# microsoft/ConfigNet

Hardware: AMD Instinct MI355X
Metric: train-step images/sec at 256x256 (G+D fwd+bwd) (higher is better)
Workload: dtype f32; 1 GPU; ConfigNet second-stage iteration (D + synth-D + latent-D + G + EMA), 256x256, batch 16 per GPU, fp32, Keras-Adam; global_batch=16, resolution=256, latent_dim=145, parallelism=dp1, losses_finite=True

## Files before the change

### confignet_amd/_lib.py

```python
import ctypes
import os

_HERE = os.path.dirname(os.path.abspath(__file__))
LIB_PATH = os.environ.get("CN_LIB") or os.path.join(_HERE, "libconfignet_hip.so")


class CnSumJob(ctypes.Structure):
    _fields_ = [("src", ctypes.c_void_p), ("dst", ctypes.c_void_p), ("count", ctypes.c_longlong), ("parts", ctypes.c_int),
                ("accumulate", ctypes.c_int)]


class CnDepthJob(ctypes.Structure):
    _fields_ = [("a", ctypes.c_void_p), ("b", ctypes.c_void_p), ("c", ctypes.c_void_p), ("m", ctypes.c_int), ("n", ctypes.c_int),
                ("k", ctypes.c_int), ("lda", ctypes.c_int), ("ldb", ctypes.c_int), ("ldc", ctypes.c_int)]


class CnRowsJob(ctypes.Structure):
    _fields_ = [("a", ctypes.c_void_p), ("b", ctypes.c_void_p), ("c", ctypes.c_void_p), ("bias", ctypes.c_void_p), ("mask", ctypes.c_void_p)] + \
               [(n_, ctypes.c_int) for n_ in ("m", "n", "k", "lda", "ldb", "ldc", "tb", "act", "accumulate")] + [("slope", ctypes.c_float)]


class CnGanJob(ctypes.Structure):
    _fields_ = [("s", ctypes.c_void_p), ("out", ctypes.c_void_p), ("gout", ctypes.c_void_p), ("n", ctypes.c_int), ("label", ctypes.c_float)]


class CnConvGeom(ctypes.Structure):
    _fields_ = [(n, ctypes.c_int) for n in (
        "nd", "n", "in_d", "in_h", "in_w", "cin", "out_d", "out_h", "out_w", "cout",
        "k_d", "k_h", "k_w", "s_d", "s_h", "s_w", "dl_d", "dl_h", "dl_w", "p_d", "p_h", "p_w", "up")]


CN_F32, CN_BF16 = 0, 1
CN_U8 = 2
CN_EUNSUPPORTED = -3


class ConfigNetHipError(RuntimeError):
    pass


if not os.path.exists(LIB_PATH):
    raise ImportError(
        "confignet_amd: %s is missing -- build it with `python confignet_amd/build.py` "
        "(or __graft_entry__.build()).  There is no CPU/PyTorch fallback." % LIB_PATH)

lib = ctypes.CDLL(LIB_PATH)

_p = ctypes.c_void_p
_i = ctypes.c_int
_f = ctypes.c_float
_z = ctypes.c_size_t
_G = ctypes.POINTER(CnConvGeom)

SIGNATURES = {
    "cn_version": [],
    "cn_conv_fwd": [_G, _p, _p, _p, _p, _i, _f, _p],
    "cn_conv_fwd_res": [_G, _p, _p, _p, _p, _p, _i, _f, _p],
    "cn_conv_fwd_stats": [_G, _p, _p, _p, _p, _i, _f, _p, _i, _f, _p],
    "cn_scale_columns_segments": [_p, _p, _p, _p, _i, _z, _p],
    "cn_conv_weight_tflip": [_p, _p, _i, _i, _i, _p],
    "cn_conv_dgrad": [_G, _p, _p, _p, _p],
    "cn_conv_dgrad_w": [_G, _p, _p, _p, _p],
    "cn_conv_dgrad_w_res": [_G, _p, _p, _p, _p, _p],
    "cn_conv_dgrad_w_mask": [_G, _p, _p, _p, _p, _p, _p, _p, _p],
    "cn_bn_fold_bwd_chunks": [],
    "cn_bn_fold_bwd": [_p, _i, _i, _p, _p, _p, _p, _p, _p, _p, _p, _i, _p],
    "cn_conv_wgrad_thin_partials": [],
    "cn_conv_wgrad_thin": [_G, _p, _p, _p, _p, _i, _p],
    "cn_conv_wgrad": [_G, _p, _p, _p, _i, _p],
    "cn_conv_wgrad_workspace_bytes": [_G],
    "cn_conv_wgrad_ws": [_G, _p, _p, _p, _i, _p, _z, _p],
    "cn_conv_wgrad_ws_slabs": [_G, _p, _p, _p, _i, _p, _z, ctypes.POINTER(_i), _p],
    "cn_conv_wgrad_dt_workspace_bytes": [_G, _i, _i, ctypes.POINTER(_z)],
    "cn_conv_wgrad_dt": [_G, _p, _i, _p, _i, _p, _i, _p, _z, ctypes.POINTER(_i), _p],
    "cn_conv_wgrad_plan": [_G, _i, _i, _i, ctypes.c_uint, _i, ctypes.POINTER(ctypes.c_longlong)],
    "cn_conv_wgrad_grouped": [_i, _p, _p, _p, _p, _p, _p, _p, _i, _p, _p],
    "cn_conv_wgrad_grouped_plan": [_i, _p, _i, _p, _p],
    "cn_sum_parts_grouped": [_p, _i, _p],
    "cn_gemm_depth_grouped": [_p, _i, _p],
    "cn_gan_loss_grouped": [_p, _i, _i, _p],
    "cn_gemm_rows_grouped": [_p, _i, _p],
    "cn_gemm_rows_grouped_k": [_p, _i, _p],
    "cn_gemm_rows_grouped_plan": [_p, _i, ctypes.POINTER(_i), _i, ctypes.POINTER(_i)],
    "cn_conv_tune": [_i, _i, ctypes.c_long],
    "cn_conv_fwd_plan": [_G, _i, _i, _i, _i, _i, _i, _i, ctypes.POINTER(ctypes.c_int * 8)],
    "cn_conv_fwd_plan_ep": [_G, _i, _i, _i, _i, _i, _i, _i, _i, ctypes.POINTER(ctypes.c_int * 8)],
    "cn_conv_loop_select": [_i, _i, _i, _i],
    "cn_fwd2_col_block": [_i, _i, _i, _i, _i, _i],
    "cn_conv_fwd_dt": [_p, _p, _i, _p, _p, _p, _i, _i, _f, _p],
    "cn_conv_dgrad_dt": [_p, _p, _i, _p, _p, _i, _p],
    "cn_conv_wgrad_c3_partials": [],
    "cn_conv_wgrad_c3": [_p, _p, _p, _i, _p, _p, _i, _p],
    "cn_conv_wino_filter": [_p, _p, _i, _i, _i, _p],
    "cn_conv_fwd_wino": [_i, _i, _i, _i, _i, _p, _p, _p, _p, _i, _f, _p],
    "cn_conv_fwd_wino_ep": [_i, _i, _i, _i, _i, _p, _p, _p, _p, _p, _p, _p],
    "cn_conv_fwd_wino4": [_i, _i, _i, _i, _i, _p, _p, _p, _p, _i, _f, _p],
    "cn_conv_fwd_wino4_ep": [_i, _i, _i, _i, _i, _p, _p, _p, _p, _i, _f, _i, _p, _p, _p, _p, _i, _f, _p],
    "cn_conv_wino4_filter": [_p, _p, _i, _i, _i, _p],
    "cn_sumpool2": [_p, _p, _i, _i, _i, _i, _i, _i, _i, _p],
    "cn_gemm": [_i, _i, _i, _i, _i, _p, _i, _p, _i, _p, _i, _p, _i, _f, _p],
    "cn_gemm_plan": [_i] * 10 + [ctypes.POINTER(ctypes.c_int * 9)],
    "cn_nc_reduce4": [_p, _p, _i, _i, _i, _f, _i, _i, _p],
    "cn_nc_reduce": [_p, _p, _p, _p, _i, _i, _i, _i, _f, _i, _p],
    "cn_nc_reduce_plan": [_i, _i, _i, _i, _i, _i, ctypes.POINTER(ctypes.c_int * 8)],
    "cn_nc_lin2": [_p, _p, _p, _p, _p, _p, _p, _p, _i, _i, _i, _i, _i, _f, _i, _p],
    "cn_nc_rows_plan": [ctypes.c_longlong, _i, _i, ctypes.POINTER(ctypes.c_int * 2)],
    "cn_norm_coef_fwd": [_i, _p, _p, _p, _p, _p, _p, _p, _p, _i, _i, _i, _f, _p, _i, _p],
    "cn_norm_coef_bwd": [_i, _p, _p, _p, _p, _p, _p, _p, _p, _p, _p, _i, _i, _i, _f, _p],
    "cn_dual_tail_coef_fwd": [_p] * 13 + [_i, _i, _i, _f, _i, _i, _p],
    "cn_dual_tail_coef_bwd": [_p] * 13 + [ctypes.POINTER(ctypes.c_void_p), _i, _i, _i, _f, _i, _i, _p],
    "cn_dual_tail_gx": [_p] * 12 + [_i, _i, _i, _f, _i, _i, _p],
    "cn_dual_tail_gx_tx": [_p] * 18 + [_i, _i, _i, _f, _i, _i, _i, _p],
    "cn_norm_apply": [_i, _i] + [_p] * 13 + [_i, _i, _i, _f, _i, _f, _i, _p],
    "cn_nc_reduce_hxt": [_p, _p, _p, _p, _i, _i, _i, _f, _i, _i, _i, _p],
    "cn_zero": [_p, ctypes.c_size_t, _p],
    "cn_set_deterministic": [_i],
    "cn_get_deterministic": [],
    "cn_det_release_stream": [_p],
    "cn_gemm_acc": [_i, _i, _i, _i, _i, _p, _i, _p, _i, _p, _i, _p],
    "cn_sum_rows_into": [_p, _p, _i, _i, _i, _p],
    "cn_bn_act_bwd": [_p, _p, _p, _p, _p, _p, _p, _p, _i, _i, _i, _i, _i, _i, _p],
    "cn_nc_reduce_dact": [_p, _p, _p, _p, _p, _i, _i, _i, _i, _f, _i, _i, _p],
    "cn_act_fwd": [_p, _p, _z, _i, _f, _i, _p],
    "cn_act_bwd": [_p, _p, _p, _z, _i, _f, _i, _p],
    "cn_act_bwd_bias": [_p, _p, _p, _p, _i, _i, _i, _i, _f, _i, _i, _p],
    "cn_axpby": [_p, _p, _p, _z, _f, _f, _i, _p],
    "cn_mul": [_p, _p, _p, _z, _i, _p],
    "cn_sqdiff_sum": [_p, _p, _p, _z, _f, _i, _p],
    "cn_row_sumsq": [_p, _p, _i, _z, _p],
    "cn_row_scale": [_p, _p, _p, _i, _z, _f, _i, _p],
    "cn_row_scale_diff": [_p, _p, _p, _p, _i, ctypes.c_size_t, _f, _i, _p],
    "cn_tap_bwd": [_p, _p, _p, _p, _p, _i, ctypes.c_size_t, _f, _i, _f, _i, _p],
    "cn_maxpool2_bwd_act": [_p, _p, _p, _p, _f, _p, _i, _i, _i, _i, _i, _i, _p],
    "cn_stream_plan": [_i, _i, ctypes.c_longlong, _z, _i, _i, _i, _i, _i, _i, ctypes.c_uint, _i, ctypes.POINTER(ctypes.c_longlong * 4)],
    "cn_stream_plan_ptrs": [_i, _i, _i, ctypes.c_longlong, _z, _i, _i, _i, _i, _i, _i, ctypes.POINTER(ctypes.c_void_p * 4), _i, ctypes.POINTER(ctypes.c_longlong * 4)],
    "cn_stream_last_plan": [ctypes.POINTER(ctypes.c_longlong * 5)],
    "cn_masked_diff": [_p, _p, _p, _p, _z, _i, _p],
    "cn_maxpool_fwd": [_p, _p, _i, _i, _i, _i, _i, _i, _i, _i, _p],
    "cn_maxpool_bwd": [_p, _p, _p, _i, _i, _i, _i, _i, _i, _i, _i, _p],
    "cn_avgpool3_same": [_p, _p, _i, _i, _i, _i, _i, _p],
    "cn_dwconv3x3_fwd": [_p, _p, _p, _p, _i, _i, _i, _i, _i, _i, _f, _p],
    "cn_image_preprocess": [_p, _i, _p, _i, _i, _i, _i, _i, _i, _f, _f, _p],
    "cn_dwconv3x3_dgrad": [_p, _p, _p, _i, _i, _i, _i, _i, _p],
    "cn_dwconv3x3_wgrad_slices": [_i, _i, _i, _i, _i],
    "cn_dwconv3x3_wgrad": [_p, _p, _p, _i, _i, _i, _i, _i, _i, _p],
    "cn_bn_train_coef": [_p] * 12 + [ctypes.c_longlong, _i, _f, ctypes.c_double, _i, _p],
    "cn_bn_train_apply": [_p, _p, _p, _p, ctypes.c_longlong, _i, _i, _p],
# ... 50 lines not shown
```

### confignet_amd/build.py

```python
import os
import subprocess
import sys

CSRC = os.path.join(os.path.dirname(os.path.abspath(__file__)), "csrc")
LIB = os.path.join(os.path.dirname(os.path.abspath(__file__)), "libconfignet_hip.so")
SOURCES = ["prof.hip", "igemm_conv.hip", "small_conv.hip", "conv_dispatch.hip", "igemm_bf16.hip", "upfold.hip", "winograd.hip", "winograd4.hip", "c3_wgrad.hip", "thin_wgrad.hip", "wgrad2.hip", "fwd2.hip", "gemm.hip", "elementwise.hip", "norm_coef.hip", "rotate3d.hip", "depthwise.hip", "bn_train.hip", "hdri.hip", "dataset.hip"]
FLAGS = ["--offload-arch=gfx950", "-O3", "-std=c++17", "-fPIC", "-munsafe-fp-atomics", "-Wall"]


def _stale(target, deps):
    if not os.path.exists(target):
        return True
    t = os.path.getmtime(target)
    return any(os.path.getmtime(d) > t for d in deps)


def build_library(force=False, verbose=True):
    hipcc = os.environ.get("HIPCC", "/opt/rocm/bin/hipcc")
    headers = [os.path.join(CSRC, f) for f in os.listdir(CSRC) if f.endswith(".h")]
    headers.append(os.path.join(os.path.dirname(CSRC), "..", "include", "confignet_hip.h"))
    objs = []
    procs = []
    for src in SOURCES:
        s = os.path.join(CSRC, src)
        o = os.path.join(CSRC, src.replace(".hip", ".o"))
        objs.append(o)
        if force or _stale(o, [s] + headers):
            cmd = [hipcc] + FLAGS + ["-c", s, "-o", o]
            if verbose:
                print(" ".join(cmd), flush=True)
            procs.append((src, subprocess.Popen(cmd)))
    for src, p in procs:
        if p.wait() != 0:
            raise RuntimeError("hipcc failed on %s" % src)
    if force or procs or _stale(LIB, objs):
        cmd = [hipcc, "--offload-arch=gfx950", "-shared", "-fPIC", "-o", LIB] + objs
        if verbose:
            print(" ".join(cmd), flush=True)
        subprocess.check_call(cmd)
    return LIB


if __name__ == "__main__":
    build_library(force="--force" in sys.argv)
    print(LIB)
```

### confignet_amd/functional.py

```python
import contextlib

import torch
from torch.autograd import Function

from . import ops
from .ops import ACT_LRELU, ACT_NONE, ACT_RELU, ACT_TANH, ConvSpec

_INPUT_GRADS_ONLY = False
FUSED_TAIL_STATS = True
FUSED_R1_TAIL = True
BN_BWD_FUSED = True


@contextlib.contextmanager
def input_grads_only():
    global _INPUT_GRADS_ONLY
    prev, _INPUT_GRADS_ONLY = _INPUT_GRADS_ONLY, True
    try:
        yield
    finally:
        _INPUT_GRADS_ONLY = prev


class _RefuseFn(Function):
# ... 19 lines not shown
    outs = list(outs)
    for i, w in zip(live, wrapped):
        outs[i] = w
    return tuple(outs)


def _cg(t):
    return t if t.is_contiguous() else t.contiguous()


def _bias_grad(gy, first_order, sink=None):
    if first_order:
        return ops.bias_grad(gy.detach(), sink=sink)
    return NcSumDotFn.apply(gy, None, True)[0].reshape(-1)


class ConvFn(Function):

    @staticmethod
    def forward(ctx, x, w, bias, spec, act, slope):
        x, w = _cg(x), _cg(w)
        g = spec.geom(tuple(x.shape), w.shape[-1])
        if ops.upfold_ok(g):
            wf, _, gd, _ = ops.upfold_prepare(w, g)
            y = ops.conv_fwd(x, wf, bias, gd, act, slope)
            ops.prof_note_saved(ops.upfold_saved_flops(g))
        else:
            y = ops.conv_fwd(x, w, bias, g, act, slope)
        ctx.save_for_backward(x, w, y if act != ACT_NONE else None)
        ctx.g, ctx.act, ctx.slope, ctx.has_bias = g, act, slope, bias is not None
        ctx.bias_ref = bias if (bias is not None and bias.requires_grad) else None
        return y

    @staticmethod
    def backward(ctx, gy):
        x, w, y = ctx.saved_tensors
        gy = _cg(gy)
        gb_fused = None
        first_order = not torch.is_grad_enabled()
        want_w = ctx.needs_input_grad[1] and not _INPUT_GRADS_ONLY
        want_b = ctx.has_bias and ctx.needs_input_grad[2] and not _INPUT_GRADS_ONLY
        w_slot = ops.sink_for(w) if (first_order and want_w) else None
        b_slot = ops.sink_for(ctx.bias_ref) if (first_order and want_b and ctx.bias_ref is not None) else None
        if ctx.act != ACT_NONE:
            if not first_order:
                raise RuntimeError("double backward through a fused-activation conv is not supported; "
                                   "use conv(..., act=ACT_NONE) + lrelu()")
            if want_b:
                gy, gb_fused = ops.act_bwd_bias(gy, y, ctx.act, ctx.slope, sink=b_slot)
            else:
                gy = ops.act_bwd(gy, y, ctx.act, ctx.slope)
        elif want_b and b_slot is not None:
            ops.bias_grad(gy.detach(), sink=b_slot)
        gx = gw = gb = None
        if want_b and b_slot is None:
            gb = gb_fused if gb_fused is not None else _bias_grad(gy, first_order)
        if ops.upfold_ok(ctx.g) and first_order:
            _, wd, _, g2 = ops.upfold_prepare(w, ctx.g)
            if ctx.needs_input_grad[0]:
                gx = ops.conv_fwd(gy, wd, None, g2)
                ops.prof_note_saved(ops.upfold_saved_flops(ctx.g))
            if want_w:
                if w_slot is not None:
                    ops.sink_upfold_wgrad(gy, x, g2, tuple(wd.shape), ctx.g, tuple(w.shape), w_slot)
                else:
                    gw = ops.upfold_wgrad(ops.conv_wgrad(gy, x, g2, tuple(wd.shape)), ctx.g, tuple(w.shape))
                ops.prof_note_saved(ops.upfold_saved_flops(ctx.g))
            return gx, gw, gb, None, None, None
        if ctx.needs_input_grad[0]:
            gx = ConvDgradFn.apply(gy, w, ctx.g)
        if want_w:
            if w_slot is not None:
                ops.sink_conv_wgrad(x, gy, ctx.g, tuple(w.shape), w_slot)
            else:
                gw = ConvWgradFn.apply(x, gy, ctx.g, tuple(w.shape))
        return gx, gw, gb, None, None, None


class ConvDgradFn(Function):

    @staticmethod
    def forward(ctx, gy, w, g):
        gy = _cg(gy)
        gu = ops.conv_dgrad(gy, w, g)
        ctx.save_for_backward(gy, w)
        ctx.g = g
        return ops.sumpool2(gu) if g.up else gu

    @staticmethod
    def backward(ctx, ggx):
        gy, w = ctx.saved_tensors
        ggx = _cg(ggx)
        g_gy = g_w = None
        if ctx.needs_input_grad[0]:
            g_gy = ConvNoBiasFromGeomFn.apply(ggx, w, ctx.g)
        if ctx.needs_input_grad[1]:
            g_w = ConvWgradFn.apply(ggx, gy, ctx.g, tuple(w.shape))
        return g_gy, g_w, None


class ConvNoBiasFromGeomFn(Function):

    @staticmethod
    def forward(ctx, x, w, g):
        x = _cg(x)
        ctx.save_for_backward(x, w)
        ctx.g = g
        return ops.conv_fwd(x, _cg(w), None, g, ACT_NONE, 0.0)

    @staticmethod
    def backward(ctx, gy):
        x, w = ctx.saved_tensors
        gy = _cg(gy)
        gx = ConvDgradFn.apply(gy, w, ctx.g) if ctx.needs_input_grad[0] else None
        gw = ConvWgradFn.apply(x, gy, ctx.g, tuple(w.shape)) if ctx.needs_input_grad[1] else None
        return gx, gw, None


class ConvWgradFn(Function):
    @staticmethod
    def forward(ctx, x, gy, g, w_shape):
        x, gy = _cg(x), _cg(gy)
        ctx.save_for_backward(x, gy)
        ctx.g, ctx.w_shape = g, w_shape
        return ops.conv_wgrad(x, gy, g, w_shape)

    @staticmethod
    def backward(ctx, ggw):
        x, gy = ctx.saved_tensors
        ggw = _cg(ggw)
        gx = ConvDgradFn.apply(gy, ggw, ctx.g) if ctx.needs_input_grad[0] else None
        ggy = ConvNoBiasFromGeomFn.apply(x, ggw, ctx.g) if ctx.needs_input_grad[1] else None
        return gx, ggy, None, None


def conv(x, w, bias, spec, act=ACT_NONE, slope=0.0):
    return ConvFn.apply(x, w, bias, spec, act, slope)


class MatmulFn(Function):

    @staticmethod
    def forward(ctx, a, b, ta, tb):
        a, b = _cg(a), _cg(b)
        ctx.save_for_backward(a, b)
        ctx.ta, ctx.tb = ta, tb
        return ops.gemm(a, b, ta, tb)

    @staticmethod
    def backward(ctx, gc):
        a, b = ctx.saved_tensors
        ta, tb = ctx.ta, ctx.tb
        ga = gb = None
        if ctx.needs_input_grad[0]:
            ga = MatmulFn.apply(b, gc, tb, True) if ta else MatmulFn.apply(gc, b, False, not tb)
        if ctx.needs_input_grad[1] and not (_INPUT_GRADS_ONLY and b.is_leaf):
            gb = MatmulFn.apply(gc, a, True, ta) if tb else MatmulFn.apply(a, gc, not ta, False)
        return ga, gb, None, None


class LinearFn(Function):

    @staticmethod
    def forward(ctx, x, w, b):
        x, w = _cg(x), _cg(w)
        ctx.save_for_backward(x, w)
        ctx.has_bias = b is not None
        ctx.bias_ref = b if (b is not None and b.requires_grad) else None
        return ops.gemm(x, w, False, False, b)
# ... 742 lines not shown
```

### confignet_amd/ops.py

```python
import contextlib
import ctypes
import math
import os
import threading

import torch

from ._lib import CN_BF16, CN_EUNSUPPORTED, CN_F32, CN_U8, CnConvGeom, CnDepthJob, CnGanJob, CnRowsJob, CnSumJob, check, lib

ACT_NONE, ACT_LRELU, ACT_RELU, ACT_TANH, ACT_RELU6, ACT_SIGMOID = 0, 1, 2, 3, 4, 5

ACT_DTYPE = torch.float32


def set_activation_dtype(dtype):
    global ACT_DTYPE
    if isinstance(dtype, str):
        dtype = {"f32": torch.float32, "fp32": torch.float32, "float32": torch.float32, "bf16": torch.bfloat16,
                 "bfloat16": torch.bfloat16}[dtype]
    assert dtype in (torch.float32, torch.bfloat16)
    ACT_DTYPE = dtype


def _stream():
# ... 383 lines not shown
def conv_dgrad_masked(gy, w, g, y, target=None, s=None, k=0.0):
    if not (ACT_DTYPE == torch.float32 and gy.dtype == torch.float32 and y.dtype == torch.float32 and _wino4_ok(g, g.cout, g.cin)):
        return None
    if target is not None and (target.dtype != torch.float32 or s is None or s.numel() not in (1, g.n)):
        return None
    _log_mask(y, ACT_RELU)
    gu = torch.empty(geom_in_shape(g, upsampled=True), device=gy.device, dtype=torch.float32)
    check(lib.cn_conv_fwd_wino4_ep(g.n, g.in_h, g.in_w, g.cout, g.cin, _ptr(_c(gy)), _ptr(_wino4_filter(w, True)), None, _ptr(gu),
                                   ACT_NONE, 0.0, W4_EP_MASK, None, _ptr(_c(y)), None if target is None else _ptr(_c(target)),
                                   None if target is None else _fptr(s), 1 if target is None else s.numel(), k, _stream()),
          "cn_conv_fwd_wino4_ep")
    prof_note_saved(wino4_saved_flops(g))
    return gu


def conv_fwd_res(x, w, bias, res, g, act=ACT_NONE, slope=0.0):
    assert act in (ACT_NONE, ACT_RELU)
    if ACT_DTYPE == torch.float32 and x.dtype == torch.float32 and res.dtype == torch.float32 and not _wino_ok(g, g.cin, g.cout):
        x, res = _c(x), _c(res)
        y = torch.empty(geom_out_shape(g), device=x.device, dtype=torch.float32)
        rc = lib.cn_conv_fwd_res(ctypes.byref(g), _ptr(x), _fptr(w), _fptr(bias), _ptr(res), _ptr(y), act, slope, _stream())
        if rc == 0:
            return y
        if rc != CN_EUNSUPPORTED:
            check(rc, "cn_conv_fwd_res")
    y = conv_fwd(x, w, bias, g)
    return nc_lin2(tuple(y.shape), y, None, res, None, None, flags=8 if act == ACT_RELU else 0)


def scale_columns_segments(src, seg, a, total):
    dst = torch.empty(total, device=src.device, dtype=torch.float32)
    check(lib.cn_scale_columns_segments(_fptr(src), _ptr(dst), _ptr(seg), _fptr(_c(a)), seg.shape[0], total, _stream()),
          "cn_scale_columns_segments")
    return dst


def weight_tflip(w):
    w = _c(w)
    taps = int(math.prod(w.shape[:-2]))
    wt = torch.empty(w.shape[:-2] + (w.shape[-1], w.shape[-2]), device=w.device, dtype=torch.float32)
    check(lib.cn_conv_weight_tflip(_fptr(w), _ptr(wt), taps, w.shape[-2], w.shape[-1], _stream()), "cn_conv_weight_tflip")
    return wt


def conv_dgrad(gy, w, g):
    shape = geom_in_shape(g, upsampled=True)
    if _bf16_conv_ok(g):
        gy = cast(gy, torch.bfloat16)
        gu = torch.empty(shape, device=gy.device, dtype=torch.bfloat16)
        _, wd = weight_prep_bf16(w)
        check(lib.cn_conv_dgrad_bf16(ctypes.byref(g), _ptr(gy), _ptr(wd), _ptr(gu), _stream()), "cn_conv_dgrad_bf16")
        return gu
    if gy.dtype == torch.bfloat16 and MIXED_FIRST_LAYERS and g.cin == 3:
        gu = torch.empty(shape, device=gy.device, dtype=torch.float32)
        wt = _weight_cache(w, "_cn_tflip", weight_tflip)
        rc = lib.cn_conv_dgrad_dt(ctypes.byref(g), _ptr(_c(gy)), CN_BF16, _fptr(wt), _ptr(gu), CN_F32, _stream())
        if rc == 0:
            return cast(gu, _act_out_dtype(g.cin))
        if rc != CN_EUNSUPPORTED:
            check(rc, "cn_conv_dgrad_dt")
    gy = f32(gy)
    gu = torch.empty(shape, device=gy.device, dtype=torch.float32)
    if ACT_DTYPE == torch.float32 and _wino4_ok(g, g.cout, g.cin):
        check(lib.cn_conv_fwd_wino4(g.n, g.in_h, g.in_w, g.cout, g.cin, _ptr(_c(gy)), _ptr(_wino4_filter(w, True)), None, _ptr(gu),
                                    ACT_NONE, 0.0, _stream()), "cn_conv_fwd_wino4")
        prof_note_saved(wino4_saved_flops(g))
        return gu
    if ACT_DTYPE == torch.float32 and _wino_ok(g, g.cout, g.cin):
        check(lib.cn_conv_fwd_wino(g.n, g.in_h, g.in_w, g.cout, g.cin, _ptr(gy), _ptr(_wino_filter(w, True)), None, _ptr(gu),
                                   ACT_NONE, 0.0, _stream()), "cn_conv_fwd_wino")
        prof_note_saved(wino_saved_flops(g))
        return gu
    if DGRAD_FROM_W:
        rc = lib.cn_conv_dgrad_w(ctypes.byref(g), _ptr(gy), _fptr(_c(w)), _ptr(gu), _stream())
        if rc == 0:
            return cast(gu, _act_out_dtype(g.cin))
        if rc != CN_EUNSUPPORTED:
            check(rc, "cn_conv_dgrad_w")
    wt = _weight_cache(w, "_cn_tflip", weight_tflip)
    check(lib.cn_conv_dgrad(ctypes.byref(g), _ptr(gy), _fptr(wt), _ptr(gu), _stream()), "cn_conv_dgrad")
    return cast(gu, _act_out_dtype(g.cin))


def conv_dgrad_res(gy, w, g, res):
    if (ACT_DTYPE == torch.float32 and gy.dtype == torch.float32 and res.dtype == torch.float32 and DGRAD_FROM_W and not g.up
            and not _wino4_ok(g, g.cout, g.cin) and not _wino_ok(g, g.cout, g.cin)):
        gu = torch.empty(geom_in_shape(g, upsampled=True), device=gy.device, dtype=torch.float32)
        rc = lib.cn_conv_dgrad_w_res(ctypes.byref(g), _ptr(_c(gy)), _fptr(_c(w)), _ptr(_c(res)), _ptr(gu), _stream())
        if rc == 0:
            return gu
        if rc != CN_EUNSUPPORTED:
            check(rc, "cn_conv_dgrad_w_res")
    gu = conv_dgrad(gy, w, g)
    return nc_lin2(tuple(gu.shape), gu, None, res, None, None)


MASK_EPILOGUE = True
MASK_LOG = None


def conv_dgrad_mask(gy, w, g, mask, res=None, sums=(), defer=True):
    assert len(sums) <= 2
    fused = None
    if (MASK_EPILOGUE and not DETERMINISTIC and ACT_DTYPE == torch.float32 and gy.dtype == torch.float32 and mask.dtype == torch.float32
            and (res is None or res.dtype == torch.float32) and DGRAD_FROM_W and not g.up and not _bf16_conv_ok(g)
            and not _wino4_ok(g, g.cout, g.cin)):
        gu = torch.empty(geom_in_shape(g, upsampled=True), device=gy.device, dtype=torch.float32)
        assert tuple(gu.shape) == tuple(mask.shape), "conv_dgrad_mask: the mask has the shape of the data gradient"
        s0 = _fptr(sums[0]) if len(sums) > 0 else None
        s1 = _fptr(sums[1]) if len(sums) > 1 else None
        if _wino_ok(g, g.cout, g.cin):
            if res is None:
                rc = lib.cn_conv_fwd_wino_ep(g.n, g.in_h, g.in_w, g.cout, g.cin, _ptr(_c(gy)), _ptr(_wino_filter(w, True)), _ptr(gu),
                                             _ptr(_c(mask)), s0, s1, _stream())
                fused = "wino"
            else:
                rc = CN_EUNSUPPORTED
        else:
            rc = lib.cn_conv_dgrad_w_mask(ctypes.byref(g), _ptr(_c(gy)), _fptr(_c(w)), None if res is None else _ptr(_c(res)),
                                          _ptr(_c(mask)), _ptr(gu), s0, s1, _stream())
            fused = "fwd2"
        if rc == 0:
            _log_mask(mask, ACT_RELU)
            if sums and _SINK is not None:
                _SINK.note_stream()
            if fused == "wino":
                prof_note_saved(wino_saved_flops(g))
            if MASK_LOG is not None:
                MASK_LOG.append(fused)
            return gu
        if rc != CN_EUNSUPPORTED:
            check(rc, "cn_conv_fwd_wino_ep" if fused == "wino" else "cn_conv_dgrad_w_mask")
        del gu
    if MASK_LOG is not None:
        MASK_LOG.append("pass")
    gu = conv_dgrad(gy, w, g) if res is None else conv_dgrad_res(gy, w, g, res)
    if not sums:
        return act_bwd(gu, mask, ACT_RELU)
    gu, part = act_bwd_partials(gu, mask, ACT_RELU)
    for dst in sums:
        sum_rows_into(part, dst, defer=defer)
    return gu


DGRAD_FROM_W = True
MIXED_FIRST_LAYERS = True
WGRAD_WRITE, WGRAD_ADD, WGRAD_ZEROED = 0, 1, 2


def conv_wgrad(x, gy, g, w_shape, out=None, accumulate=True, defer=True, ws=None):
    gw, mode = out, WGRAD_ADD if accumulate else WGRAD_WRITE
    if out is None:
        gw, mode = zero_pool_alloc(w_shape, x.device), WGRAD_ZEROED
        if gw is None:
            gw, mode = torch.empty(w_shape, device=x.device, dtype=torch.float32), WGRAD_WRITE
    x = _c(cast(x, torch.bfloat16 if _bf16_conv_ok(g) else torch.float32))
    nbytes = ctypes.c_size_t(0)
    rc = lib.cn_conv_wgrad_dt_workspace_bytes(ctypes.byref(g), _dt(x), _dt(gy), ctypes.byref(nbytes))
    if rc == CN_EUNSUPPORTED and gy.dtype != x.dtype:
        gy = cast(gy, x.dtype)
        rc = lib.cn_conv_wgrad_dt_workspace_bytes(ctypes.byref(g), _dt(x), _dt(gy), ctypes.byref(nbytes))
    check(rc, "cn_conv_wgrad_dt_workspace_bytes")
    gy, nbytes = _c(gy), nbytes.value
    if ws is None:
        ws = torch.empty(nbytes // 4, device=x.device, dtype=torch.float32) if nbytes else None
    else:
# ... 1084 lines not shown
```

### include/confignet_hip.h

```cpp
#ifndef CONFIGNET_HIP_H
#define CONFIGNET_HIP_H
#include <stddef.h>
#include <stdint.h>

#ifdef __cplusplus
extern "C" {
#endif

#define CN_OK 0
#define CN_EINVAL (-1)
#define CN_EHIP (-2)
#define CN_EUNSUPPORTED (-3)

#define CN_F32 0
#define CN_BF16 1
#define CN_U8 2

#define CN_ACT_NONE 0
#define CN_ACT_LRELU 1
#define CN_ACT_RELU 2
#define CN_ACT_TANH 3
#define CN_ACT_RELU6 4
#define CN_ACT_SIGMOID 5

// ... 23 lines not shown
int cn_conv_dgrad_w_res(const CnConvGeom* g, const float* gy, const float* w, const float* res, float* gu, void* stream);
int cn_conv_dgrad_w_mask(const CnConvGeom* g, const float* gy, const float* w, const float* res, const float* mask, float* gu,
                         float* colsum, float* colsum2, void* stream);
int cn_conv_wgrad(const CnConvGeom* g, const float* x, const float* gy, float* gw, int accumulate, void* stream);
size_t cn_conv_wgrad_workspace_bytes(const CnConvGeom* g);
int cn_conv_wgrad_ws(const CnConvGeom* g, const float* x, const float* gy, float* gw, int accumulate, void* workspace,
                     size_t workspace_bytes, void* stream);
int cn_conv_wgrad_ws_slabs(const CnConvGeom* g, const float* x, const float* gy, float* gw, int accumulate, void* workspace,
                           size_t workspace_bytes, int* parts, void* stream);
#define CN_WGRAD_WRITE 0
#define CN_WGRAD_ADD 1
#define CN_WGRAD_ZEROED 2
int cn_conv_wgrad_dt_workspace_bytes(const CnConvGeom* g, int x_dt, int gy_dt, size_t* bytes);
int cn_conv_wgrad_dt(const CnConvGeom* g, const void* x, int x_dt, const void* gy, int gy_dt, float* gw, int mode, void* workspace,
                     size_t workspace_bytes, int* parts, void* stream);
int cn_conv_wgrad_plan(const CnConvGeom* g, int x_dt, int gy_dt, int caller_slabs, unsigned routes, int det, long long out[12]);
int cn_conv_wgrad_grouped(int njobs, const CnConvGeom* geoms, const float* const* x, const float* const* gy, float* const* out,
                          float* const* ws, const size_t* ws_bytes, const int* accumulate, int solo, int* parts, void* stream);
int cn_conv_wgrad_grouped_plan(int njobs, const CnConvGeom* geoms, int solo, long long* out, long long info[4]);
typedef struct CnSumJob {
    const float* src;
    float* dst;
    long long count;
    int parts;
    int accumulate;
} CnSumJob;
int cn_sum_parts_grouped(const CnSumJob* jobs, int njobs, void* stream);
typedef struct CnDepthJob {
    const float* a;
    const float* b;
    float* c;
    int m, n, k, lda, ldb, ldc;
} CnDepthJob;
int cn_gemm_depth_grouped(const CnDepthJob* jobs, int njobs, void* stream);
typedef struct CnRowsJob {
    const float* a;
    const float* b;
    float* c;
    const float* bias;
    const float* mask;
    int m, n, k, lda, ldb, ldc, tb, act, accumulate;
    float slope;
} CnRowsJob;
int cn_gemm_rows_grouped(const CnRowsJob* jobs, int njobs, void* stream);
int cn_gemm_rows_grouped_k(const CnRowsJob* jobs, int njobs, void* stream);
int cn_gemm_rows_grouped_plan(const CnRowsJob* jobs, int njobs, int* out, int cap, int* nlaunches);
typedef struct CnGanJob {
    const float* s;
    float* out;
    const float* gout;
    int n;
    float label;
} CnGanJob;
int cn_gan_loss_grouped(const CnGanJob* jobs, int njobs, int backward, void* stream);
int cn_conv_fwd_dt(const CnConvGeom* g, const void* x, int x_dt, const float* w, const float* bias, void* y, int y_dt, int act,
                   float slope, void* stream);
int cn_conv_dgrad_dt(const CnConvGeom* g, const void* gy, int gy_dt, const float* w_tflip, void* gu, int gu_dt, void* stream);
int cn_conv_wgrad_c3_partials(void);
int cn_conv_wgrad_c3(const CnConvGeom* g, const float* x, const void* gy, int gy_dt, float* scratch, float* gw, int accumulate,
                     void* stream);
int cn_conv_wgrad_thin_partials(void);
int cn_conv_wgrad_thin(const CnConvGeom* g, const float* x, const float* gy, float* scratch, float* gw, int accumulate, void* stream);
int cn_conv_wino_filter(const float* w, float* u, int cin, int cout, int dgrad, void* stream);
int cn_conv_fwd_wino(int n, int h, int w, int cin, int cout, const float* x, const float* u, const float* bias, float* y,
                     int act, float slope, void* stream);
int cn_conv_fwd_wino_ep(int n, int h, int w, int cin, int cout, const float* x, const float* u, float* y, const float* mask,
                        float* colsum, float* colsum2, void* stream);
int cn_conv_wino4_filter(const float* w, float* u, int cin, int cout, int dgrad, void* stream);
int cn_conv_fwd_wino4(int n, int h, int w, int cin, int cout, const float* x, const float* u, const float* bias,
                      float* y, int act, float slope, void* stream);
#define CN_W4_EP_POOL 1
#define CN_W4_EP_POOL_ONLY 2
#define CN_W4_EP_MASK 3
int cn_conv_fwd_wino4_ep(int n, int h, int w, int cin, int cout, const float* x, const float* u, const float* bias, float* y,
                         int act, float slope, int mode, float* pooled, const float* ym, const float* target, const float* s,
                         int s_rows, float k, void* stream);
int cn_conv_tune(int cfg, int splits, long wg_blocks);
int cn_conv_fwd_plan(const CnConvGeom* g, int bt, int has_bias, int act, int has_res, int stats_mode, int x_dt, int y_dt, int out[8]);
int cn_conv_fwd_plan_ep(const CnConvGeom* g, int bt, int has_bias, int act, int has_res, int stats_mode, int has_mask, int x_dt, int y_dt,
                        int out[8]);
int cn_conv_loop_select(int loop, int kb, int ns, int np);
int cn_fwd2_col_block(int cfg, int bt, int gathered, int n, int kb, int np);
int cn_sumpool2(const void* gu, void* gx, int nd, int n, int d, int h, int w, int c, int dt, void* stream);

int cn_conv_weight_prep_bf16(const float* w, uint16_t* wf, uint16_t* wd, int taps, int cin, int cout, void* stream);
int cn_conv_fwd_bf16(const CnConvGeom* g, const uint16_t* x, const uint16_t* wf, const float* bias, uint16_t* y,
                     int act, float slope, void* stream);
int cn_conv_dgrad_bf16(const CnConvGeom* g, const uint16_t* gy, const uint16_t* wd, uint16_t* gu, void* stream);
int cn_conv_wgrad_bf16(const CnConvGeom* g, const uint16_t* x, const uint16_t* gy, float* gw, int accumulate, void* stream);
int cn_upfold_weights(const float* w, float* wf, float* wd, int nd, const int* k3, const int* pad_lo3, int cin, int cout,
                      int* k2_out3, int* pad2_out3, void* stream);
int cn_upfold_wgrad(const float* gw2, float* gw, int nd, const int* k3, const int* pad_lo3, int cin, int cout,
                    int accumulate, void* stream);
int cn_cast(const void* src, int src_dt, void* dst, int dst_dt, size_t numel, void* stream);

int cn_gemm(int trans_a, int trans_b, int m, int n, int k, const float* a, int lda,
            const float* b, int ldb, float* c, int ldc, const float* bias, int act, float slope,
            void* stream);
int cn_gemm_plan(int trans_a, int trans_b, int m, int n, int k, int ldc, int has_bias, int act, int accumulate, int deterministic,
                 int out[9]);

int cn_set_deterministic(int on);
int cn_get_deterministic(void);
int cn_det_release_stream(void* stream);
int cn_zero(void* p, size_t bytes, void* stream);
int cn_gemm_acc(int trans_a, int trans_b, int m, int n, int k, const float* a, int lda, const float* b, int ldb,
                float* c, int ldc, void* stream);
int cn_sum_rows_into(const float* src, float* dst, int rows, int cols, int accumulate, void* stream);

int cn_nc_reduce_plan(int n, int s, int c, int nsums, int prezeroed, int det, int out[8]);
int cn_nc_reduce4(const void* x, float* out, int n, int s, int c, float slope, int flags, int dt, void* stream);
int cn_nc_reduce(const void* x1, const void* x2, float* sum1, float* sum2, int n, int s, int c,
                 int flags, float slope, int dt, void* stream);
int cn_nc_reduce_dact(const void* x1, const void* x2, float* sum1, float* sum2, void* dact_out, int n, int s, int c,
                      int flags, float slope, int act, int dt, void* stream);
int cn_bn_act_bwd(const void* gy, const void* y, const void* x, const float* a, void* g_out, void* gx, float* sum_g,
                  float* sum_gx, int n, int s, int c, int act, int flags, int dt, void* stream);
int cn_nc_lin2(const void* x1, const float* a1, const void* x2, const float* a2, const float* bb,
               const float* a3, const float* b3, void* y, int n, int s, int c, int cstride, int flags,
               float slope, int dt, void* stream);
int cn_nc_rows_plan(long long G, int CG, int ny, int out[2]);

int cn_norm_coef_fwd(int mode, const float* s1, const float* s2, const float* p1, const float* p2, float* A,
                     float* B, float* save_mean, float* save_r, int n, int c, int S, float eps, const void* x, int dt,
                     void* stream);
int cn_norm_coef_bwd(int mode, const float* t1, const float* t2, const float* save_mean, const float* save_r,
                     const float* p1, float* c1, float* c2, float* c0, float* gp1, float* gp2, int n, int c,
                     int S, float eps, void* stream);
int cn_norm_apply(int mode, int dir, const void* x1, const void* x2, const float* sa, const float* sb, const float* p1,
                  const float* p2, float* save_mean, float* save_r, float* gp1, float* gp2, const float* a3, const float* b3,
                  void* y, int n, int s, int c, float eps, int flags, float slope, int dt, void* stream);

int cn_dual_tail_coef_fwd(const float* T1, const float* T2, const float* U1, const float* U2, const float* mean,
                          const float* q, const float* sm, const float* ssd, const float* gamma, float* C1,
                          float* C2, float* C0, float* tstyle, int n, int c, int S, float eps, int n_style, int period,
                          void* stream);
int cn_dual_tail_coef_bwd(const float* H1, const float* H2p, const float* E, const float* u, const float* T1,
                          const float* T2, const float* U1, const float* U2, const float* mean, const float* q,
                          const float* sm, const float* ssd, const float* gamma, float* const* out13, int n, int c,
                          int S, float eps, int n_style, int period, void* stream);
int cn_dual_tail_gx(const void* h, const void* ta, const void* tx, const void* x, const float* kh,
                    const float* kt, const float* ka, const float* kc, const float* et, const float* ex,
                    const float* e0, void* out, int n, int s, int c, float slope, int nrep, int dt, void* stream);
int cn_dual_tail_gx_tx(const void* h, const void* ta, const void* tx, const void* x, const float* kh, const float* kt,
                       const float* ka, const float* kc, const float* et, const float* ex, const float* e0,
                       const float* K1, const float* K2, const float* K0, const float* D2, const float* D0, void* out,
                       void* out_tx, int n, int s, int c, float slope, int nrep, int ta_is_tx, int dt, void* stream);
int cn_nc_reduce_hxt(const void* h, const void* x, const void* ta, float* out, int n, int s, int c, float slope, int period,
                     int flags, int dt, void* stream);

int cn_act_fwd(const void* x, void* y, size_t numel, int act, float slope, int dt, void* stream);
int cn_act_bwd(const void* gy, const void* y, void* gx, size_t numel, int act, float slope, int dt, void* stream);
int cn_act_bwd_bias(const void* gy, const void* y, void* gx, float* gb, int n, int s, int c, int act, float slope, int flags,
                    int dt, void* stream);
int cn_axpby(const void* x, const void* y, void* out, size_t numel, float a, float b, int dt, void* stream);
int cn_mul(const void* x, const void* y, void* out, size_t numel, int dt, void* stream);
int cn_sqdiff_sum(const void* a, const void* b, float* out, size_t numel, float scale, int dt, void* stream);
int cn_row_sumsq(const float* x, float* out, int n, size_t row, void* stream);
int cn_row_scale(const void* x, const float* s, void* out, int n, size_t row, float k, int dt, void* stream);
int cn_row_scale_diff(const void* x, const void* x2, const float* s, void* out, int n, size_t row, float k, int dt, void* stream);
int cn_tap_bwd(const void* y, const void* target, const void* g, const float* s, void* out, int n, size_t row, float k,
               int act, float slope, int dt, void* stream);
int cn_maxpool2_bwd_act(const void* x, const void* gy, const void* target, const float* s, float k, void* gx, int n, int h,
                        int w, int c, int s_rows, int dt, void* stream);
int cn_stream_plan(int op, int dt, long long rows, size_t row, int c, int h, int w, int k, int s, int pad, unsigned aligned, int det,
                   long long out[4]);
// ... 73 lines not shown
```

Measured before the change: 449.1 images/sec.

## Add fused upsample-conv dgrad kernel for 4x4 RGB-output layers

Adds a specialized HIP kernel that computes the input gradient of a nearest-upsample-by-2 followed by a 4x4 conv with few output channels (1-4). It folds the sum-pool into effective 5x5 weights built in shared memory, so it avoids the full-resolution dgrad plus a separate sumpool2 pass. ConvDgradFn uses the kernel whenever the upsample geometry matches and falls back to the old path otherwise. The kernel is used only in double-backward paths such as R1, and it adds shared-memory-heavy tiles whose occupancy is a risk.

```diff
diff --git a/confignet_amd/_lib.py b/confignet_amd/_lib.py
--- a/confignet_amd/_lib.py
+++ b/confignet_amd/_lib.py
@@ -63,6 +63,7 @@
     "cn_conv_dgrad_w": [_G, _p, _p, _p, _p],
     "cn_conv_dgrad_w_res": [_G, _p, _p, _p, _p, _p],
     "cn_conv_dgrad_w_mask": [_G, _p, _p, _p, _p, _p, _p, _p, _p],
+    "cn_conv_dgrad_up2k4_rgb": [_G, _p, _i, _p, _p, _p],
     "cn_bn_fold_bwd_chunks": [],
     "cn_bn_fold_bwd": [_p, _i, _i, _p, _p, _p, _p, _p, _p, _p, _p, _i, _p],
     "cn_conv_wgrad_thin_partials": [],
diff --git a/confignet_amd/build.py b/confignet_amd/build.py
--- a/confignet_amd/build.py
+++ b/confignet_amd/build.py
@@ -4,7 +4,7 @@
 
 CSRC = os.path.join(os.path.dirname(os.path.abspath(__file__)), "csrc")
 LIB = os.path.join(os.path.dirname(os.path.abspath(__file__)), "libconfignet_hip.so")
-SOURCES = ["prof.hip", "igemm_conv.hip", "small_conv.hip", "conv_dispatch.hip", "igemm_bf16.hip", "upfold.hip", "winograd.hip", "winograd4.hip", "c3_wgrad.hip", "thin_wgrad.hip", "wgrad2.hip", "fwd2.hip", "gemm.hip", "elementwise.hip", "norm_coef.hip", "rotate3d.hip", "depthwise.hip", "bn_train.hip", "hdri.hip", "dataset.hip"]
+SOURCES = ["prof.hip", "igemm_conv.hip", "small_conv.hip", "conv_dispatch.hip", "igemm_bf16.hip", "upfold.hip", "up2k4_dgrad.hip", "winograd.hip", "winograd4.hip", "c3_wgrad.hip", "thin_wgrad.hip", "wgrad2.hip", "fwd2.hip", "gemm.hip", "elementwise.hip", "norm_coef.hip", "rotate3d.hip", "depthwise.hip", "bn_train.hip", "hdri.hip", "dataset.hip"]
 FLAGS = ["--offload-arch=gfx950", "-O3", "-std=c++17", "-fPIC", "-munsafe-fp-atomics", "-Wall"]
 
 
diff --git a/confignet_amd/csrc/up2k4_dgrad.hip b/confignet_amd/csrc/up2k4_dgrad.hip
--- /dev/null
+++ b/confignet_amd/csrc/up2k4_dgrad.hip
@@ -0,0 +1,135 @@
+#include "common.h"
+
+namespace {
+
+constexpr int UD_TW = 64, UD_PG = 8, UD_PW = 2 * UD_TW + 3;
+constexpr int UD_RS = 140;
+constexpr int UD_THREADS = 256;
+
+template <int CO>
+__global__ __launch_bounds__(UD_THREADS) void up2k4_rgb_dgrad_kernel(const float* __restrict__ GY, const float* __restrict__ W,
+                                                                    float* __restrict__ GX, int H, int Wd, int C, int TH, int ph, int pw) {
+    extern __shared__ __align__(16) float lds[];
+    const int PR = 2 * TH + 3;
+    float* S = lds;
+    float* patch = lds + 25 * CO * C;
+    const int tid = threadIdx.x;
+    const int tiles_w = (Wd + UD_TW - 1) / UD_TW, tiles_h = (H + TH - 1) / TH;
+    int b = blockIdx.x;
+    const int tj = b % tiles_w; b /= tiles_w;
+    const int ti = b % tiles_h;
+    const int n = b / tiles_h;
+    const int i0 = ti * TH, j0 = tj * UD_TW;
+    const int H2 = 2 * H, W2 = 2 * Wd;
+    const int r0 = 2 * i0 + ph - 3, q0 = 2 * j0 + pw - 3;
+    constexpr int UD_B = 4;
+    for (int base = tid; base < 25 * CO * C; base += UD_B * UD_THREADS) {
+        float wv[UD_B][4];
+#pragma unroll
+        for (int u = 0; u < UD_B; ++u) {
+            const int idx = min(base + u * UD_THREADS, 25 * CO * C - 1);
+            const int ci = idx % C;
+            int r = idx / C;
+            const int co = r % CO; r /= CO;
+            const int e = r / 5, f = r - e * 5;
+            const int kh0 = max(0, 3 - e), kw0 = max(0, 3 - f);
+            const bool h2 = kh0 + 1 <= min(3, 4 - e), w2 = kw0 + 1 <= min(3, 4 - f);
+            const int kh1 = h2 ? kh0 + 1 : kh0, kw1 = w2 ? kw0 + 1 : kw0;
+            const float a = W[((kh0 * 4 + kw0) * C + ci) * CO + co], b = W[((kh0 * 4 + kw1) * C + ci) * CO + co];
+            const float c = W[((kh1 * 4 + kw0) * C + ci) * CO + co], d = W[((kh1 * 4 + kw1) * C + ci) * CO + co];
+            wv[u][0] = a; wv[u][1] = w2 ? b : 0.f; wv[u][2] = h2 ? c : 0.f; wv[u][3] = (h2 && w2) ? d : 0.f;
+        }
+#pragma unroll
+        for (int u = 0; u < UD_B; ++u) {
+            const int idx = base + u * UD_THREADS;
+            if (idx < 25 * CO * C) S[idx] = ((wv[u][0] + wv[u][1]) + wv[u][2]) + wv[u][3];
+        }
+    }
+    const float* gsrc = GY + (long)n * H2 * W2 * CO;
+    for (int base = tid; base < PR * UD_PW * CO; base += UD_B * UD_THREADS) {
+        float gv[UD_B];
+        int dst[UD_B];
+#pragma unroll
+        for (int u = 0; u < UD_B; ++u) {
+            const int idx = base + u * UD_THREADS;
+            const int rr = idx / (UD_PW * CO), k = idx - rr * (UD_PW * CO);
+            const int c = k / CO, co = k - c * CO;
+            const int gr = r0 + rr, gc = q0 + c;
+            const bool in = idx < PR * UD_PW * CO && gr >= 0 && gr < H2 && gc >= 0 && gc < W2;
+            const float v = gsrc[in ? ((long)gr * W2 + gc) * CO + co : 0];
+            gv[u] = in ? v : 0.f;
+            dst[u] = idx < PR * UD_PW * CO ? (co * PR + rr) * UD_RS + c + (c >> 4) : -1;
+        }
+#pragma unroll
+        for (int u = 0; u < UD_B; ++u)
+            if (dst[u] >= 0) patch[dst[u]] = gv[u];
+    }
+    __syncthreads();
+    const int NG = C >> 2;
+    const float4* S4 = reinterpret_cast<const float4*>(S);
+    for (int item = tid; item < TH * UD_PG * NG; item += UD_THREADS) {
+        const int cg = item % NG;
+        int r = item / NG;
+        const int pg = r % UD_PG, li = r / UD_PG;
+        float4 acc[UD_PG];
+#pragma unroll
+        for (int q = 0; q < UD_PG; ++q) acc[q] = make_float4(0.f, 0.f, 0.f, 0.f);
+#pragma unroll 1
+        for (int e = 0; e < 5; ++e) {
+#pragma unroll
+            for (int co = 0; co < CO; ++co) {
+                const float* row = patch + (co * PR + 2 * li + e) * UD_RS + 17 * pg;
+                float gv[2 * UD_PG + 3];
+#pragma unroll
+                for (int k = 0; k < 2 * UD_PG + 3; ++k) gv[k] = row[k + (k >> 4)];
+                float4 sf[5];
+#pragma unroll
+                for (int f = 0; f < 5; ++f) sf[f] = S4[((e * 5 + f) * CO + co) * NG + cg];
+#pragma unroll
+                for (int f = 0; f < 5; ++f)
+#pragma unroll
+                    for (int q = 0; q < UD_PG; ++q) {
+                        const float v = gv[2 * q + f];
+                        acc[q].x += v * sf[f].x; acc[q].y += v * sf[f].y; acc[q].z += v * sf[f].z; acc[q].w += v * sf[f].w;
+                    }
+            }
+        }
+        const int i = i0 + li;
+        if (i >= H) continue;
+        float* dst = GX + (((long)n * H + i) * Wd + j0 + UD_PG * pg) * C + 4 * cg;
+#pragma unroll
+        for (int q = 0; q < UD_PG; ++q)
+            if (j0 + UD_PG * pg + q < Wd) *reinterpret_cast<float4*>(dst + (long)q * C) = acc[q];
+    }
+}
+
+}
+
+extern "C" int cn_conv_dgrad_up2k4_rgb(const CnConvGeom* g, const void* gy, int gy_dt, const float* w, float* gx, void* stream) {
+    CN_CHECK_ARG(g && gy && w && gx, "cn_conv_dgrad_up2k4_rgb: NULL argument");
+    if (g->nd != 2 || g->up != 1 || g->k_h != 4 || g->k_w != 4 || g->s_h != 1 || g->s_w != 1 || g->dl_h != 1 || g->dl_w != 1)
+        return CN_EUNSUPPORTED;
+    if (g->p_h != 1 || g->p_w != 1 || g->out_h != 2 * g->in_h || g->out_w != 2 * g->in_w || g->n < 1 || g->in_h < 1 || g->in_w < 1)
+        return CN_EUNSUPPORTED;
+    if (g->cout < 1 || g->cout > 4 || g->cin < 4 || g->cin % 4 || g->cin > 64 || gy_dt != CN_F32 || cn_det()) return CN_EUNSUPPORTED;
+    const int TH = g->cin >= 32 ? 4 : 8;
+    const long tiles = (long)g->n * cn_cdiv(g->in_h, TH) * cn_cdiv(g->in_w, UD_TW);
+    if (tiles > 0x7fffffffL) return CN_EUNSUPPORTED;
+    const size_t lds = sizeof(float) * ((size_t)25 * g->cout * g->cin + (size_t)g->cout * (2 * TH + 3) * UD_RS);
+    hipStream_t s = (hipStream_t)stream;
+    cn_prof_begin(s, 2.0 * 25.0 * g->cout * g->n * g->in_h * g->in_w * g->cin,
+                  4.0 * g->n * g->in_h * g->in_w * (4.0 * g->cout + g->cin), CN_FAM_THIN);
+#define UD_LAUNCH(CO_)                                                                                                             \
+    hipLaunchKernelGGL((up2k4_rgb_dgrad_kernel<CO_>), dim3((unsigned)tiles), dim3(UD_THREADS), lds, s, (const float*)gy, w, gx, g->in_h, \
+                       g->in_w, g->cin, TH, g->p_h, g->p_w)
+    switch (g->cout) {
+        case 1: UD_LAUNCH(1); break;
+        case 2: UD_LAUNCH(2); break;
+        case 3: UD_LAUNCH(3); break;
+        default: UD_LAUNCH(4); break;
+    }
+#undef UD_LAUNCH
+    cn_prof_end(s);
+    CN_LAUNCH_CHECK();
+    return CN_OK;
+}
diff --git a/confignet_amd/functional.py b/confignet_amd/functional.py
--- a/confignet_amd/functional.py
+++ b/confignet_amd/functional.py
@@ -125,9 +125,12 @@
     @staticmethod
     def forward(ctx, gy, w, g):
         gy = _cg(gy)
-        gu = ops.conv_dgrad(gy, w, g)
         ctx.save_for_backward(gy, w)
         ctx.g = g
+        gx = ops.conv_dgrad_up2k4(gy, w, g) if g.up else None
+        if gx is not None:
+            return gx
+        gu = ops.conv_dgrad(gy, w, g)
         return ops.sumpool2(gu) if g.up else gu
 
     @staticmethod
diff --git a/confignet_amd/ops.py b/confignet_amd/ops.py
--- a/confignet_amd/ops.py
+++ b/confignet_amd/ops.py
@@ -489,6 +489,21 @@
     return cast(gu, _act_out_dtype(g.cin))
 
 
+UP2K4_DGRAD = True
+
+
+def conv_dgrad_up2k4(gy, w, g):
+    if not (UP2K4_DGRAD and g.up and ACT_DTYPE == torch.float32 and gy.dtype == torch.float32 and w.dtype == torch.float32
+            and not DETERMINISTIC):
+        return None
+    gx = torch.empty(geom_in_shape(g), device=gy.device, dtype=torch.float32)
+    rc = lib.cn_conv_dgrad_up2k4_rgb(ctypes.byref(g), _ptr(_c(gy)), CN_F32, _fptr(_c(w)), _ptr(gx), _stream())
+    if rc == CN_EUNSUPPORTED:
+        return None
+    check(rc, "cn_conv_dgrad_up2k4_rgb")
+    return gx
+
+
 def conv_dgrad_res(gy, w, g, res):
     if (ACT_DTYPE == torch.float32 and gy.dtype == torch.float32 and res.dtype == torch.float32 and DGRAD_FROM_W and not g.up
             and not _wino4_ok(g, g.cout, g.cin) and not _wino_ok(g, g.cout, g.cin)):
diff --git a/include/confignet_hip.h b/include/confignet_hip.h
--- a/include/confignet_hip.h
+++ b/include/confignet_hip.h
@@ -129,6 +129,7 @@
 int cn_conv_loop_select(int loop, int kb, int ns, int np);
 int cn_fwd2_col_block(int cfg, int bt, int gathered, int n, int kb, int np);
 int cn_sumpool2(const void* gu, void* gx, int nd, int n, int d, int h, int w, int c, int dt, void* stream);
+int cn_conv_dgrad_up2k4_rgb(const CnConvGeom* g, const void* gy, int gy_dt, const float* w, float* gx, void* stream);
 
 int cn_conv_weight_prep_bf16(const float* w, uint16_t* wf, uint16_t* wd, int taps, int cin, int cout, void* stream);
 int cn_conv_fwd_bf16(const CnConvGeom* g, const uint16_t* x, const uint16_t* wf, const float* bias, uint16_t* y,
```

Result: no change. 451.6 images/sec, median of 6 (+0.5%).
